# HumanCompatibleAI/imitation

Measured on NVIDIA H100. Metric: GAIL env-steps/sec (disc+gen loop), higher is better.
Workload: dtype f32

## Files before the change

imitation_b200/csrc/imb_ppo.cu:

```cuda
#include <cooperative_groups.h>
#include <stdlib.h>

#include "imb_common.cuh"
#include "imb_tile.cuh"

#ifdef IMB_PPO_TIMING
__device__ long long g_ppo_clk[24];
__device__ long long g_ppo_wclk[80];
#define PPO_TICK(i)                                  \
  do {                                               \
    if (tid == 0) {                                  \
      const long long now_ = clock64();              \
      clk_acc[i] += now_ - clk_last;                 \
      clk_last = now_;                               \
    }                                                \
  } while (0)
#define PPO_WCLK(slot)                                   \
  do {                                                   \
    if (lane == 0) wacc[slot] += clock64() - wclk0;      \
  } while (0)
#else
#define PPO_TICK(i) do {} while (0)
#define PPO_WCLK(slot) do {} while (0)
#endif
// ... 81 lines not shown
__device__ __forceinline__ float group8_sum(float v) {
  v += __shfl_xor_sync(0xffffffffu, v, 1);
  v += __shfl_xor_sync(0xffffffffu, v, 2);
  v += __shfl_xor_sync(0xffffffffu, v, 4);
  return v;
}
__device__ __forceinline__ float rcp_fast(float x) { return __fdividef(1.0f, x); }
__device__ __forceinline__ float sqrt_fast(float x) {
  float r;
  asm("sqrt.approx.f32 %0, %1;" : "=f"(r) : "f"(x));
  return r;
}

__device__ __forceinline__ float dot8r(const float (&d)[8], const float* __restrict__ b) {
  const float4 b0 = ld4(b), b1 = ld4(b + 4);
  float s0 = d[0] * b0.x, s1 = d[1] * b0.y;
  s0 = fmaf(d[2], b0.z, s0);
  s1 = fmaf(d[3], b0.w, s1);
  s0 = fmaf(d[4], b1.x, s0);
  s1 = fmaf(d[5], b1.y, s1);
  s0 = fmaf(d[6], b1.z, s0);
  s1 = fmaf(d[7], b1.w, s1);
  return s0 + s1;
}
__device__ __forceinline__ void load8(float (&d)[8], const float* __restrict__ p) {
  const float4 a = ld4(p), b = ld4(p + 4);
  d[0] = a.x, d[1] = a.y, d[2] = a.z, d[3] = a.w, d[4] = b.x, d[5] = b.y, d[6] = b.z, d[7] = b.w;
}
__device__ __forceinline__ float sum8(const float (&d)[8]) {
  return ((d[0] + d[1]) + (d[2] + d[3])) + ((d[4] + d[5]) + (d[6] + d[7]));
}

enum { RS_PG = 0, RS_V, RS_ENT, RS_CLIP, RS_KL, RS_N };
enum { AC_PG = 0, AC_V, AC_ENT, AC_CLIP, AC_KL_EPOCH, AC_LAST_PG, AC_LAST_V, AC_LAST_ENT, AC_N };

template <int NR>
__device__ __forceinline__ void ppo_stats_fold(float* __restrict__ acc, const float* __restrict__ rsl, const float inv_nb,
                                               const bool epoch_start) {
#pragma unroll 1
  for (int k = 0; k < RS_N; ++k) {
    float t = 0.f;
#pragma unroll
    for (int r = 0; r < NR; ++r) t += rsl[k * NR + r];
    t *= inv_nb;
    if (k == RS_KL) {
      acc[AC_KL_EPOCH] = epoch_start ? t : acc[AC_KL_EPOCH] + t;
    } else {
      acc[k] += t;
      if (k < RS_CLIP) acc[AC_LAST_PG + k] = t;
    }
  }
}

__device__ __forceinline__ void ppo_stats_fold_warp(float* __restrict__ acc, const float* __restrict__ rsl,
                                                    const float inv_nb, const bool epoch_start, const int lane) {
  static_assert(RS_CLIP == 3 && RS_KL == 4 && RL == 8, "fold layout");
  const float a = group8_sum(rsl[lane]), kl = group8_sum(rsl[RS_KL * RL + (lane & 7)]) * inv_nb;
  const float s_v = __shfl_sync(0xffffffffu, a, 8), s_ent = __shfl_sync(0xffffffffu, a, 16);
  const float s_clip = __shfl_sync(0xffffffffu, a, 24);
  if (lane == 0) {
    const float pg = a * inv_nb, v = s_v * inv_nb, ent = s_ent * inv_nb;
    acc[AC_PG] += pg;
    acc[AC_V] += v;
    acc[AC_ENT] += ent;
    acc[AC_CLIP] += s_clip * inv_nb;
    acc[AC_KL_EPOCH] = epoch_start ? kl : acc[AC_KL_EPOCH] + kl;
    acc[AC_LAST_PG] = pg;
    acc[AC_LAST_V] = v;
    acc[AC_LAST_ENT] = ent;
  }
}

template <int NR>
__device__ __forceinline__ float ppo_kl_part(const float* __restrict__ rsl, const float inv_nb) {
  float t = 0.f;
#pragma unroll
  for (int r = 0; r < NR; ++r) t += rsl[RS_KL * NR + r];
  return t * inv_nb;
}

__device__ __noinline__ void ppo_ev_partial(const float* __restrict__ rollout, const int64_t N, const int rw,
                                            const int col_val, const int col_ret, const int crank, double* ev,
                                            double* wred) {
  const int tid = threadIdx.x, lane = tid & 31, warp = tid >> 5;
  const double y0 = rollout[col_ret], e0 = rollout[col_ret] - rollout[col_val];
  double s[4] = {0.0, 0.0, 0.0, 0.0};
  for (int64_t i = (int64_t)crank * PT + tid; i < N; i += (int64_t)CL * PT) {
    const float y = rollout[i * rw + col_ret], e = y - rollout[i * rw + col_val];
    const double dy = (double)y - y0, de = (double)e - e0;
    s[0] += dy;
    s[1] += dy * dy;
    s[2] += de;
    s[3] += de * de;
  }
#pragma unroll
  for (int k = 0; k < 4; ++k) {
    double v = s[k];
#pragma unroll
    for (int o = 16; o > 0; o >>= 1) v += __shfl_xor_sync(0xffffffffu, v, o);
    __syncthreads();
    if (lane == 0) wred[warp] = v;
    __syncthreads();
    if (tid == 0) {
      double t = 0.0;
#pragma unroll
      for (int w = 0; w < PT / 32; ++w) t += wred[w];
      ev[k] = t;
    }
  }
}

template <typename Cluster>
__device__ __forceinline__ void ppo_stats_push(Cluster& cluster, float* box, const float* acc, const double* ev,
                                               const int crank) {
  float* dst = cluster.map_shared_rank(box, 0) + crank * 16;
#pragma unroll
  for (int k = 0; k < AC_N; ++k) dst[k] = acc[k];
#pragma unroll
  for (int k = 0; k < 4; ++k) reinterpret_cast<double*>(dst + 8)[k] = ev[k];
}

__device__ __noinline__ void ppo_stats_finish(const float* box, float* __restrict__ stats, const PpoArgs& A,
                                              const int64_t n_eval, const int64_t n_epochs, const int64_t spe,
                                              const float std, const int64_t n_updates, const bool stopped) {
  float acc[AC_N];
  double ev[4] = {0.0, 0.0, 0.0, 0.0};
#pragma unroll
  for (int k = 0; k < AC_N; ++k) acc[k] = 0.f;
  for (int c = 0; c < CL; ++c) {
    const float* a = box + c * 16;
    const double* e = reinterpret_cast<const double*>(box + c * 16 + 8);
#pragma unroll
    for (int k = 0; k < AC_N; ++k) acc[k] += a[k];
#pragma unroll
    for (int k = 0; k < 4; ++k) ev[k] += e[k];
  }
  const float ne = (float)n_eval;
  stats[IMB_PPO_STAT_ENTROPY_LOSS] = acc[AC_ENT] / ne;
  stats[IMB_PPO_STAT_PG_LOSS] = acc[AC_PG] / ne;
  stats[IMB_PPO_STAT_VALUE_LOSS] = acc[AC_V] / ne;
  stats[IMB_PPO_STAT_APPROX_KL] = acc[AC_KL_EPOCH] / (float)((n_eval - 1) % spe + 1);
  stats[IMB_PPO_STAT_CLIP_FRACTION] = acc[AC_CLIP] / ne;
  stats[IMB_PPO_STAT_LOSS] = acc[AC_LAST_PG] + A.hp.ent_coef * acc[AC_LAST_ENT] + A.hp.vf_coef * acc[AC_LAST_V];
  const double n = (double)A.n_rows;
  const double var_y = ev[1] / n - (ev[0] / n) * (ev[0] / n), var_e = ev[3] / n - (ev[2] / n) * (ev[2] / n);
  stats[IMB_PPO_STAT_EXPLAINED_VARIANCE] = var_y == 0.0 ? __int_as_float(0x7fc00000) : (float)(1.0 - var_e / var_y);
  stats[IMB_PPO_STAT_STD] = std;
  stats[IMB_PPO_STAT_N_UPDATES] = (float)n_updates;
  stats[IMB_PPO_STAT_N_STEPS] = (float)n_eval;
  stats[IMB_PPO_STAT_N_EPOCHS] = (float)n_epochs;
  stats[IMB_PPO_STAT_STOPPED] = stopped ? 1.f : 0.f;
}

struct WgradOff {
  int w1, b1, w2, b2, wa, ba, wv, bv, ls, ldo, ldh;
};
template <int NQ, int HPx>
__device__ __forceinline__ void tower_wgrad(const int tnet, const int gj, const int wq, const int h, const int Do, const int Da,
                                            const bool discrete, const WgradOff o, float* __restrict__ GP,
                                            const float* __restrict__ tH1, const float* __restrict__ tLAT,
                                            const float* __restrict__ tDZ2, const float* __restrict__ tDZ1,
                                            const float* __restrict__ XNc, const float* __restrict__ DM,
                                            const float* __restrict__ DLS, const float* __restrict__ DVAL) {
  constexpr int RLc = 8;
  constexpr int T2 = (HPx + NQ - 1) / NQ;
  float dz2[8], dz1[8], lt[8];
  if (gj < h) {
    load8(dz2, tDZ2 + gj * RLc);
    load8(dz1, tDZ1 + gj * RLc);
    load8(lt, tLAT + gj * RLc);
    {
      float r[T2];
#pragma unroll
      for (int t = 0; t < T2; ++t) {
        const int i = wq + NQ * t;
        r[t] = dot8r(dz2, tH1 + (i < HPx ? i : 0) * RLc);
      }
#pragma unroll
      for (int t = 0; t < T2; ++t) {
        const int i = wq + NQ * t;
        if (i < h) GP[o.w2 + gj * o.ldh + i] = r[t];
      }
    }
#pragma unroll
    for (int kb = 0; kb < Do; kb += 4 * NQ) {
      const int k0 = kb + wq;
      if (k0 >= Do) break;
      float r[4];
#pragma unroll
      for (int t = 0; t < 4; ++t) {
        const int k = k0 + NQ * t;
        r[t] = dot8r(dz1, XNc + (k < Do ? k : 0) * RLc);
      }
#pragma unroll
      for (int t = 0; t < 4; ++t) {
        const int k = k0 + NQ * t;
        if (k < Do) GP[o.w1 + gj * o.ldo + k] = r[t];
      }
    }
    if (tnet == 0) {
#pragma unroll
      for (int ab = 0; ab < Da; ab += 2 * NQ) {
        const int a0 = ab + wq, a1 = a0 + NQ;
        if (a0 >= Da) break;
        const float ra = dot8r(lt, DM + a0 * RLc), rb = dot8r(lt, DM + (a1 < Da ? a1 : a0) * RLc);
        GP[o.wa + a0 * o.ldh + gj] = ra;
        if (a1 < Da) GP[o.wa + a1 * o.ldh + gj] = rb;
      }
    } else if (wq == 0) {
      GP[o.wv + gj] = dot8r(lt, DVAL);
    }
    if (wq == 0) GP[o.b2 + gj] = sum8(dz2);
    if (wq == NQ - 1) GP[o.b1 + gj] = sum8(dz1);
  }
  if (wq == NQ - 1) {
    if (tnet == 0) {
#pragma unroll
      for (int tb = 0; tb < 2 * Da; tb += HPx) {
        const int t = tb + gj;
        if (t >= 2 * Da) break;
        if (t < Da) {
          load8(dz2, DM + t * RLc);
          GP[o.ba + t] = sum8(dz2);
        } else if (!discrete) {
          load8(dz2, DLS + (t - Da) * RLc);
          GP[o.ls + t - Da] = sum8(dz2);
        }
      }
    } else if (gj == 0) {
      load8(dz2, DVAL);
      GP[o.bv] = sum8(dz2);
    }
  }
}

template <int HP, int DO = 0, int DA = 0, int DISC = 0, int NORM = 0, int OPT = 0>
__global__ void __launch_bounds__(PT, 1) k_ppo_update(const PpoArgs A, float* __restrict__ g_params,
                                                      float* __restrict__ g_norm, int32_t* __restrict__ g_norm_count,
                                                      float* __restrict__ g_m, float* __restrict__ g_v,
                                                      const float* __restrict__ rollout,
                                                      const int64_t* __restrict__ perm_in,
                                                      float* __restrict__ loss_log, int64_t* __restrict__ state) {
  static_assert(HP == 32, "the warp-autonomous chain maps one lane to one hidden unit");
  namespace cg = cooperative_groups;
  cg::cluster_group cluster = cg::this_cluster();
  const int crank = (int)cluster.block_rank();
  extern __shared__ __align__(128) float smem[];
  __shared__ float red[32];
  __shared__ float bc[8];
  __shared__ __align__(8) uint64_t mbar[3];
  __shared__ __align__(8) uint64_t xbar[3];
  __shared__ float SSQ[CL];
  __shared__ float nred[PT / 32];
  __shared__ float RSL[RS_N * RL];
  __shared__ float ACC[AC_N];
  __shared__ float KLS[CL];
  __shared__ int KSTOP;
  __shared__ double EVP[4];
  __shared__ double EVW[PT / 32];
  const imb_policy_desc& pd = A.pol;
  constexpr bool SPEC = DO != 0;
  const int Do = SPEC ? DO : pd.d_obs, Da = SPEC ? DA : pd.d_act, h = SPEC ? HP : pd.hidden, NP = pd.n_params;
  const bool discrete = SPEC ? DISC != 0 : pd.discrete != 0, has_norm = SPEC ? NORM != 0 : pd.has_norm != 0;
  const PLay PL = make_play(Do, Da, h, discrete);
  const int KP = SPEC ? ppo_kp(Do) : A.KP, S = SPEC ? ppo_slice(PL) : A.S;
  constexpr int U_DO = SPEC ? DO : 8, U_H = SPEC ? HP : 8, U_DA = SPEC ? DA : 4;
  const int n_own_w = (S / 4 + 31) / 32;
  const bool tail_stats = n_own_w <= PT / 32 - 2;
  const int st0 = tail_stats ? 32 * max(n_own_w, 4) : 128, nst = PT - st0;
  const int ldo = PL.ldo, ldh = PL.ldh;
  const int da_store = discrete ? 1 : Da;
  const int col_logp = Do + da_store, col_adv = col_logp + 3, col_ret = col_logp + 4;
  const int tid = threadIdx.x, lane = tid & 31, warp = tid >> 5;
  const int rw = SPEC ? imb_row_width(Do, Da, discrete) : A.rw, RS2 = SPEC ? ppo_row_stride(rw) : A.RS2;
  auto al = [](int x) { return (x + 31) / 32 * 32; };
  const bool kl_on = OPT && A.target_kl > 0.f, vf_on = OPT && A.clip_vf > 0.f;

  int o = 0;
  float* Pm = smem + o; o += al(CL * S);
  float* Ms = smem + o; o += al(CL * S);
  float* Vs = smem + o; o += al(CL * S);
  float* GP = smem + o; o += al(CL * S);
  float* RECV = smem + o; o += al(CL * S);
  float* LOSS = smem + o; o += 32;
  const int DAP = (Da + 3) / 4 * 4;
  const int rsz = al(PR * RS2);
  float* ROWS = smem + o; o += 3 * rsz;
  const int xsz = al(KP * RL);
  float* XNo = smem + o; o += 2 * xsz;
  float* TH1 = smem + o; o += 2 * HP * RL;
  float* TLAT = smem + o; o += 2 * HP * RL;
  float* TDZ2 = smem + o; o += 2 * HP * RL;
  float* TDZ1 = smem + o; o += 2 * HP * RL;
  float* DM = smem + o; o += DAP * RL;
  float* DLS = smem + o; o += DAP * RL;
  float* MEAN = smem + o; o += DAP * RL;
  float* DVAL = smem + o; o += 32;
  float* rstat = smem + o; o += al(2 * 64 + 4);

  for (int i = tid; i < CL * S; i += PT) Pm[i] = Ms[i] = Vs[i] = GP[i] = RECV[i] = 0.f;
  for (int i = tid; i < 3 * rsz; i += PT) ROWS[i] = 0.f;
  for (int i = tid; i < 2 * xsz + 8 * HP * RL + 3 * DAP * RL + 32; i += PT) XNo[i] = 0.f;
  if (tid < 64) {
    rstat[tid] = (has_norm && tid < Do) ? g_norm[tid] : 0.f;
    rstat[64 + tid] = (has_norm && tid < Do) ? g_norm[Do + tid] : 1.f;
    LOSS[tid & 31] = 0.f;
  }
  if (tid < RS_N * RL) RSL[tid] = 0.f;
  if (tid < AC_N) ACC[tid] = 0.f;
  if (tid == 0) {
    KSTOP = 0;
    mbar_init(&mbar[0], nst);
    mbar_init(&mbar[1], nst);
    mbar_init(&mbar[2], nst);
    mbar_init(&xbar[0], 1);
    mbar_init(&xbar[1], 1);
    mbar_init(&xbar[2], 1);
    mbar_fence_init();
  }
  __syncthreads();
  for (int p = tid; p < NP; p += PT) {
    const int q = flat_to_play(pd, PL, p);
    Pm[q] = g_params[p];
    Ms[q] = g_m[p];
    Vs[q] = g_v[p];
  }
  int32_t run_count = has_norm ? *g_norm_count : 0;

  const int64_t N = A.n_rows;
  const int Ni = (int)N;
  const int mb = A.hp.batch_size;
  const int64_t steps_per_epoch = (N + mb - 1) / mb;
  const int64_t n_steps = steps_per_epoch * A.hp.n_epochs;
  int64_t adam_step = state[IMB_ST_PPO_STEP];
  const int64_t perm_draw0 = state[IMB_ST_PPO_EPOCH];
  double b1pow = pow(0.9, (double)adam_step), b2pow = pow(0.999, (double)adam_step);
  const int row0 = crank * RL;
  const WgradOff wo_p = {PL.w1[0], PL.b1[0], PL.w2[0], PL.b2[0], PL.wa, PL.ba, PL.wv, PL.bv, PL.ls, ldo, ldh};
  const WgradOff wo_v = {PL.w1[1], PL.b1[1], PL.w2[1], PL.b2[1], PL.wa, PL.ba, PL.wv, PL.bv, PL.ls, ldo, ldh};

  auto issue_gather = [&](int ep, int start, int buf) {
    if (tid < st0) return;
    const int nbx = min(mb, Ni - start);
#pragma unroll
    for (int tb = 0; tb < 2 * PR; tb += nst) {
      const int t = tb + tid - st0, r = t >> 1, half = t & 1;
      if (t >= 2 * PR) break;
      if (r >= nbx) continue;
      int64_t idx;
      if (perm_in) {
        idx = perm_in[(int64_t)ep * N + start + r];
      } else {
        const FeistelKey fk = feistel_key(A.seed, IMB_STREAM_PPO_PERM, (uint64_t)(perm_draw0 + ep), (uint64_t)N);
        idx = (int64_t)feistel_perm(fk, (uint64_t)(start + r), (uint64_t)N);
      }
      const float* src = rollout + idx * rw;
      float* dst = ROWS + buf * rsz + r * RS2;
      const int nq = rw >> 2, q0 = half ? (nq + 1) >> 1 : 0, q1 = half ? nq : (nq + 1) >> 1;
#pragma unroll
      for (int qi = 0; qi < (nq + 1) >> 1; ++qi) {
        const int q = q0 + qi;
        if (q >= q1) break;
        cp_async16(dst + 4 * q, src + 4 * q);
      }
    }
    cp_async_mbar_arrive(&mbar[buf]);
  };
  auto minibatch_stats = [&](int64_t gs2, int nbx, int gidx, int ngrp) {
    const int buf = (int)(gs2 % 3);
    float* R = ROWS + buf * rsz;
    float* XN = XNo + (int)(gs2 & 1) * xsz;
    const int gl = tid & 7;
    const float inv_nbx = 1.0f / (float)nbx;
    mbar_wait(&mbar[buf], (uint32_t)((gs2 / 3) & 1));
#pragma unroll
    for (int task0 = 0; task0 <= Do; task0 += ngrp) {
      const int task = task0 + gidx;
      const bool is_feat = task < Do, is_adv = task == Do;
      float* x = R + (is_feat ? task : col_adv);
      float v[8], s = 0.f;
#pragma unroll
      for (int i = 0; i < 8; ++i) {
        v[i] = (gl + 8 * i < nbx) ? x[(gl + 8 * i) * RS2] : 0.f;
        s += v[i];
      }
      const float bmean = group8_sum(s) * inv_nbx;
      float q = 0.f;
#pragma unroll
      for (int i = 0; i < 8; ++i) {
        const float d = (gl + 8 * i < nbx) ? v[i] - bmean : 0.f;
        q = fmaf(d, d, q);
      }
      const float ssd = group8_sum(q);
      if (is_feat) {
        float mean = 0.f, istd = 1.f;
        if (has_norm) {
          mean = rstat[task];
          float var = rstat[64 + task];
          const float bvar = ssd * inv_nbx;
          const float bn = (float)nbx, c = (float)run_count, itot = rcp_fast(c + bn), delta = bmean - mean;
          mean += delta * bn * itot;
          var *= c;
          var += bvar * bn;
          var += delta * delta * c * bn * itot;
          var *= itot;
          istd = rsqrtf(var + pd.norm_eps);
          if (gl == 0) {
            if (kl_on && crank == 0 && gs2 > 0) {
              g_norm[task] = rstat[task];
              g_norm[Do + task] = rstat[64 + task];
            }
            rstat[task] = mean;
            rstat[64 + task] = var;
          }
        }
        XN[task * RL + gl] = (row0 + gl < nbx) ? (x[(row0 + gl) * RS2] - mean) * istd : 0.f;
      } else if (is_adv) {
        float am = 0.f, ais = 1.f;
        if (A.hp.normalize_advantage && nbx > 1) {
          am = bmean;
          ais = rcp_fast(sqrt_fast(ssd / (float)(nbx - 1)) + 1e-8f);
        }
#pragma unroll
        for (int i = 0; i < 8; ++i)
          if (gl + 8 * i < nbx) x[(gl + 8 * i) * RS2] = (v[i] - am) * ais;
      }
    }
  };
  __syncthreads();
  issue_gather(0, 0, 0);
  if (n_steps > 1) issue_gather(mb >= Ni ? 1 : 0, mb >= Ni ? 0 : mb, 1);
  if (A.stats) ppo_ev_partial(rollout, N, rw, col_logp + 1, col_ret, crank, EVP, EVW);
  minibatch_stats(0, min(mb, Ni), tid >> 3, PT / 8);
  if (has_norm) run_count += min(mb, Ni);
  const uint32_t xbytes = (uint32_t)((CL - 1) * S * 4);
  const unsigned qmagic = (unsigned)(0x100000000ull / (unsigned)(S / 4)) + 1u;
  const uint32_t recv_sa = smem_u32(RECV), pm_sa = smem_u32(Pm), ssq_sa = smem_u32(SSQ);
  const uint32_t xbar0_sa = smem_u32(&xbar[0]), xbar1_sa = smem_u32(&xbar[1]), xbar2_sa = smem_u32(&xbar[2]);
  const uint32_t nbytes = (uint32_t)(CL * 4 * (kl_on ? 2 : 1));
  if (tid == 0) {
    mbar_expect_tx(&xbar[0], xbytes);
    mbar_expect_tx(&xbar[1], xbytes);
    mbar_expect_tx(&xbar[2], nbytes);
  }
  cluster.sync();

#ifdef IMB_PPO_TIMING
  long long clk_acc[16] = {0}, clk_last = clock64();
  long long wacc[10] = {0};
#endif
  int ep_now = 0, start = 0;
  for (int64_t gs = 0; gs < n_steps; ++gs) {
    const int cur = (int)(gs & 1);
    const float* Rc = ROWS + (int)(gs % 3) * rsz;
    const float* XNc = XNo + cur * xsz;
    const int nb = min(mb, Ni - start);
    const float inv_nb = 1.0f / (float)nb;
    int ep_next = ep_now, start_next = start + mb;
    if (start_next >= Ni) {
      start_next = 0;
      ++ep_next;
    }
    ++adam_step;
    if (tid == PT - 1) {
      b1pow *= 0.9;
      b2pow *= 0.999;
      bc[2 * cur] = (float)((double)A.hp.lr / (1.0 - b1pow));
      bc[2 * cur + 1] = (float)sqrt(1.0 - b2pow);
    }
    __syncthreads();
    if (kl_on && KSTOP) {
      if (tid >= st0 && gs + 1 < n_steps) mbar_wait(&mbar[(int)((gs + 1) % 3)], (uint32_t)(((gs + 1) / 3) & 1));
      if (has_norm) run_count -= min(mb, Ni - start);
      break;
    }
    PPO_TICK(0);
#ifdef IMB_PPO_TIMING
    const long long wclk0 = clock64();
#endif
    float l_pg = 0.f, l_v = 0.f, l_ent = 0.f;
    auto next_stats = [&]() {
      if (gs + 1 < n_steps) minibatch_stats(gs + 1, min(mb, Ni - start_next), (tid - st0) >> 3, nst / 8);
      PPO_WCLK(1);
    };
    if (warp >= 4) {
      if (tid >= st0) {
        if (!tail_stats) next_stats();
        if (gs + 2 < n_steps) {
          int ep2 = ep_next, start2 = start_next + mb;
          if (start2 >= Ni) {
            start2 = 0;
            ++ep2;
// ... 66 lines not shown
      st4(cLAT + j * RL + r0, make_float4(lat0, lat1, lat2, lat3));
      PPO_WCLK(4);
      float dl0 = 0.f, dl1 = 0.f, dl2 = 0.f, dl3 = 0.f;
      auto oct_sum = [&](float v) {
        v += __shfl_xor_sync(0xffffffffu, v, 4);
        v += __shfl_xor_sync(0xffffffffu, v, 2);
        v += __shfl_xor_sync(0xffffffffu, v, 1);
        return v;
      };
      if (cnet == 1) {
        const float wvj = jl ? Pm[PL.wv + j] : 0.f;
        const float p0 = lat0 * wvj, p1 = lat1 * wvj, p2 = lat2 * wvj, p3 = lat3 * wvj;
        const bool up16 = (lane & 16) != 0, up8 = (lane & 8) != 0;
        float k0 = up16 ? p2 : p0, k1 = up16 ? p3 : p1;
        k0 += __shfl_xor_sync(0xffffffffu, up16 ? p0 : p2, 16);
        k1 += __shfl_xor_sync(0xffffffffu, up16 ? p1 : p3, 16);
        float kk = up8 ? k1 : k0;
        kk += __shfl_xor_sync(0xffffffffu, up8 ? k0 : k1, 8);
        const float val = oct_sum(kk) + Pm[PL.bv];
        float dv;
        bool vin = true;
        if (vf_on) {
          const float vold = row[col_logp + 1], dvo = val - vold;
          dv = (vold + fminf(fmaxf(dvo, -A.clip_vf), A.clip_vf)) - row[col_ret];
          vin = dvo >= -A.clip_vf && dvo <= A.clip_vf;
        } else {
          dv = val - row[col_ret];
        }
        const float dval = (live && vin) ? A.hp.vf_coef * 2.0f * dv * inv_nb : 0.f;
        if (la == 0) {
          if (live) l_v = dv * dv;
          DVAL[r0 + rr] = dval;
          RSL[RS_V * RL + r0 + rr] = live ? dv * dv : 0.f;
        }
        dl0 = __shfl_sync(0xffffffffu, dval, 0) * wvj;
        dl1 = __shfl_sync(0xffffffffu, dval, 8) * wvj;
        dl2 = __shfl_sync(0xffffffffu, dval, 16) * wvj;
        dl3 = __shfl_sync(0xffffffffu, dval, 24) * wvj;
      } else {
        const float* Wa = Pm + PL.wa;
        __syncwarp();
        {
          const int asub = lane >> 2, q = lane & 3;
          const bool b0 = (lane & 1) != 0, b1 = (lane & 2) != 0;
#pragma unroll
          for (int ab = 0; ab < Da; ab += 8) {
            const int a = ab + asub, ac = a < Da ? a : 0;
            const float* wr = Wa + ac * ldh + q;
            const float* lr = cLAT + q * RL + r0;
            float s0 = 0.f, s1 = 0.f, s2 = 0.f, s3 = 0.f;
#pragma unroll
            for (int i = 0; i < HP / 4; ++i) {
              const float w = wr[4 * i];
              const float4 l4 = ld4(lr + 4 * i * RL);
              s0 = fmaf(w, l4.x, s0);
              s1 = fmaf(w, l4.y, s1);
              s2 = fmaf(w, l4.z, s2);
              s3 = fmaf(w, l4.w, s3);
            }
            float ka = b0 ? s1 : s0, kb = b0 ? s3 : s2;
            ka += __shfl_xor_sync(0xffffffffu, b0 ? s0 : s1, 1);
            kb += __shfl_xor_sync(0xffffffffu, b0 ? s2 : s3, 1);
            float kk = b1 ? kb : ka;
            kk += __shfl_xor_sync(0xffffffffu, b1 ? ka : kb, 2);
            if (a < Da) MEAN[a * RL + r0 + q] = kk + Pm[PL.ba + a];
          }
        }
        __syncwarp();
        PPO_WCLK(5);
        const float adv = pre_adv, logp_old = pre_lpo;
        float logp = 0.f, ent = 0.f;
        float r_dm = 0.f, r_dls = 0.f;
        int act = 0;
        if (gfast) {
          if (la < Da) {
            const float diff = pre_act - MEAN[la * RL + r0 + rr];
            const float d2 = diff * diff * pre_ivar;
            logp = -0.5f * d2 - pre_ls - 0.9189385332046727f;
            ent = 1.4189385332046727f + pre_ls;
            r_dm = diff * pre_ivar;
            r_dls = d2 - 1.0f;
          }
        } else if (!discrete) {
          const float* lstd = Pm + PL.ls;
          for (int a = la; a < Da; a += 8) {
            const float ls = lstd[a], ivar = __expf(-2.0f * ls);
            const float diff = row[Do + a] - MEAN[a * RL + r0 + rr];
            const float d2 = diff * diff * ivar;
            logp += -0.5f * d2 - ls - 0.9189385332046727f;
            ent += 1.4189385332046727f + ls;
            DM[a * RL + r0 + rr] = diff * ivar;
            DLS[a * RL + r0 + rr] = d2 - 1.0f;
          }
        } else {
          float mx = -INFINITY;
          for (int a = la; a < Da; a += 8) mx = fmaxf(mx, MEAN[a * RL + r0 + rr]);
          mx = fmaxf(mx, __shfl_xor_sync(0xffffffffu, mx, 4));
          mx = fmaxf(mx, __shfl_xor_sync(0xffffffffu, mx, 2));
          mx = fmaxf(mx, __shfl_xor_sync(0xffffffffu, mx, 1));
          float se = 0.f;
          for (int a = la; a < Da; a += 8) se += expf(MEAN[a * RL + r0 + rr] - mx);
          const float lse = mx + logf(oct_sum(se));
          act = (int)row[Do];
          for (int a = la; a < Da; a += 8) {
            const float lp = MEAN[a * RL + r0 + rr] - lse;
            if (a == act) logp = lp;
            ent -= expf(lp) * lp;
            DLS[a * RL + r0 + rr] = lp;
          }
        }
        logp = oct_sum(logp);
        PPO_WCLK(6);
        ent = oct_sum(ent);
        const float ratio = __expf(logp - logp_old);
        const float lo = 1.0f - A.hp.clip_range, hi = 1.0f + A.hp.clip_range;
        const float pl1 = adv * ratio, pl2 = adv * fminf(fmaxf(ratio, lo), hi);
        const bool inside = (ratio >= lo) && (ratio <= hi);
        float dl_dlogp = (inside || pl1 < pl2) ? -adv * ratio * inv_nb : 0.f;
        float dent = -A.hp.ent_coef * inv_nb;
        if (live) {
          if (la == 0) {
            l_pg = -fminf(pl1, pl2);
            l_ent = -ent;
          }
        } else {
          dl_dlogp = 0.f;
          dent = 0.f;
        }
        if (la == 0) {
          const int sr = r0 + rr;
          RSL[RS_PG * RL + sr] = live ? -fminf(pl1, pl2) : 0.f;
          RSL[RS_ENT * RL + sr] = live ? -ent : 0.f;
          RSL[RS_CLIP * RL + sr] = (live && fabsf(ratio - 1.0f) > A.hp.clip_range) ? 1.f : 0.f;
          RSL[RS_KL * RL + sr] = live ? (ratio - 1.0f) - (logp - logp_old) : 0.f;
        }
        if (gfast) {
          if (la < Da) {
            DLS[la * RL + r0 + rr] = dl_dlogp * r_dls + dent;
            DM[la * RL + r0 + rr] = dl_dlogp * r_dm;
          }
        } else if (!discrete) {
          for (int a = la; a < Da; a += 8) {
            DLS[a * RL + r0 + rr] = dl_dlogp * DLS[a * RL + r0 + rr] + dent;
            DM[a * RL + r0 + rr] = dl_dlogp * DM[a * RL + r0 + rr];
          }
        } else {
          for (int a = la; a < Da; a += 8) {
            const float lp = DLS[a * RL + r0 + rr], pp = expf(lp);
            DM[a * RL + r0 + rr] = dl_dlogp * (((a == act) ? 1.f : 0.f) - pp) + dent * (-pp * (lp + ent));
            DLS[a * RL + r0 + rr] = 0.f;
          }
        }
        __syncwarp();
        PPO_WCLK(7);
#pragma unroll U_DA
        for (int a = 0; a < Da; ++a) {
          const float waj = Wa[a * ldh + jc];
          const float4 d = ld4(DM + a * RL + r0);
          dl0 = fmaf(d.x, waj, dl0);
          dl1 = fmaf(d.y, waj, dl1);
          dl2 = fmaf(d.z, waj, dl2);
          dl3 = fmaf(d.w, waj, dl3);
        }
      }
      PPO_WCLK(2);
      st4(cDZ2 + j * RL + r0,
          make_float4(jl ? dl0 * (1.0f - lat0 * lat0) : 0.f, jl ? dl1 * (1.0f - lat1 * lat1) : 0.f,
                      jl ? dl2 * (1.0f - lat2 * lat2) : 0.f, jl ? dl3 * (1.0f - lat3 * lat3) : 0.f));
      __syncwarp();
      a0 = a1 = a2 = a3 = 0.f;
      {
        const float* wp = cW2 + jc;
#pragma unroll U_H
        for (int jj = 0; jj < h; ++jj) {
          const float w = wp[jj * ldh];
          const float4 d = ld4(cDZ2 + jj * RL + r0);
          a0 = fmaf(d.x, w, a0);
          a1 = fmaf(d.y, w, a1);
          a2 = fmaf(d.z, w, a2);
          a3 = fmaf(d.w, w, a3);
        }
      }
      st4(cDZ1 + j * RL + r0,
          make_float4(jl ? a0 * (1.f - h10 * h10) : 0.f, jl ? a1 * (1.f - h11 * h11) : 0.f,
                      jl ? a2 * (1.f - h12 * h12) : 0.f, jl ? a3 * (1.f - h13 * h13) : 0.f));
    }
    PPO_WCLK(0);
    if (warp >= 2) {
      asm volatile("bar.sync 1, 192;" ::: "memory");
      tower_wgrad<6, HP>(1, lane, warp - 2, h, Do, Da, discrete, wo_v, GP, TH1 + HP * RL, TLAT + HP * RL,
                         TDZ2 + HP * RL, TDZ1 + HP * RL, XNc, DM, DLS, DVAL);
    }
    PPO_WCLK(8);
    if (loss_log) {
      const float s_pg = block_sum(l_pg, red);
      const float s_v = block_sum(l_v, red);
      const float s_ent = block_sum(l_ent, red);
      if (tid == 0) {
        float* L0 = cluster.map_shared_rank(LOSS, 0);
        L0[crank * 3 + 0] = s_pg;
        L0[crank * 3 + 1] = s_v;
        L0[crank * 3 + 2] = s_ent;
      }
    }
    __syncthreads();
    PPO_TICK(3);
    tower_wgrad<PT / 32, HP>(0, lane, warp, h, Do, Da, discrete, wo_p, GP, TH1, TLAT, TDZ2, TDZ1, XNc, DM, DLS, DVAL);
    __syncthreads();
    PPO_TICK(7);
#pragma unroll
    for (int qb = 0; qb < (CL - 1) * (S / 4); qb += PT) {
      const int q = qb + tid;
      if (q >= (CL - 1) * (S / 4)) break;
      int qq = q + ((crank + 1) & (CL - 1)) * (S / 4);
      if (qq >= CL * S / 4) qq -= CL * S / 4;
      const int p0 = 4 * qq, owner = SPEC ? qq / (S / 4) : (int)__umulhi((unsigned)qq, qmagic);
      st_async_v4(mapa_u32(recv_sa + (uint32_t)(crank * S + (p0 - owner * S)) * 4u, owner), ld4(GP + p0),
                  mapa_u32(xbar0_sa, owner));
    }
    if (loss_log) cluster.sync();
    if (crank == 0 && tid == 0 && loss_log) {
      float pg = 0.f, vl = 0.f, el = 0.f;
      for (int c = 0; c < CL; ++c) {
        pg += LOSS[c * 3 + 0];
        vl += LOSS[c * 3 + 1];
        el += LOSS[c * 3 + 2];
      }
      pg *= inv_nb, vl *= inv_nb, el *= inv_nb;
      loss_log[gs * 4 + 0] = pg;
      loss_log[gs * 4 + 1] = vl;
      loss_log[gs * 4 + 2] = el;
      loss_log[gs * 4 + 3] = pg + A.hp.ent_coef * el + A.hp.vf_coef * vl;
    }
    PPO_TICK(8);
    if (A.stats && warp == ((tail_stats && n_own_w < 4) ? 3 : PT / 32 - 1))
      ppo_stats_fold_warp(ACC, RSL, rcp_fast((float)min(mb, Ni - start)), start == 0, threadIdx.x & 31);
    if (tail_stats && tid >= st0) {
      next_stats();
    } else {
      mbar_wait(&xbar[0], (uint32_t)(gs & 1));
      if (tid == 0) mbar_expect_tx(&xbar[0], xbytes);
      PPO_TICK(9);

      const int i0 = 4 * tid;
      const bool own = i0 < S;
      float4 g = make_float4(0.f, 0.f, 0.f, 0.f);
      float ss = 0.f;
      if (own) {
        auto part = [&](int c) { return ld4(c == crank ? GP + crank * S + i0 : RECV + c * S + i0); };
        g = part(0);
  #pragma unroll
        for (int c = 1; c < CL; ++c) {
          const float4 t = part(c);
          g.x += t.x, g.y += t.y, g.z += t.z, g.w += t.w;
        }
        ss = (g.x * g.x + g.y * g.y) + (g.z * g.z + g.w * g.w);
      }
      float my_ssq = 0.f;
      if (warp < n_own_w) {
        const float ws = warp_sum(ss);
        if (lane == 0) nred[warp] = ws;
        asm volatile("bar.sync 2, %0;" ::"r"(32 * n_own_w) : "memory");
  #pragma unroll
        for (int w = 0; w < PT / 32; ++w) my_ssq += w < n_own_w ? nred[w] : 0.f;
      }
      if (tid < CL) {
        st_async_f32(mapa_u32(ssq_sa + (uint32_t)crank * 4u, tid), my_ssq, mapa_u32(xbar2_sa, tid));
        if (kl_on)
          st_async_f32(mapa_u32(smem_u32(KLS) + (uint32_t)crank * 4u, tid), ppo_kl_part<RL>(RSL, inv_nb),
                       mapa_u32(xbar2_sa, tid));
      }
      PPO_TICK(10);
      mbar_wait(&xbar[2], (uint32_t)(gs & 1));
      if (tid == 0) mbar_expect_tx(&xbar[2], nbytes);
      PPO_TICK(11);
      bool stop = false;
      if (kl_on) {
        float kl = 0.f;
#pragma unroll
        for (int c = 0; c < CL; ++c) kl += KLS[c];
        stop = kl > 1.5f * A.target_kl;
        if (stop && tid == 0) KSTOP = (int)gs + 1;
      }

      float total = 0.f;
  #pragma unroll
      for (int c = 0; c < CL; ++c) total += SSQ[c];
      total = sqrtf(total);
      float clip = A.hp.max_grad_norm / (total + 1e-6f);
      clip = clip > 1.0f ? 1.0f : clip;
      if (own && !stop) {
        const float step_size = bc[2 * cur], inv_bc2s = rcp_fast(bc[2 * cur + 1]);
        const int q0 = crank * S + i0;
        const float4 m4 = ld4(Ms + q0), v4 = ld4(Vs + q0), p4 = ld4(Pm + q0);
        auto adam1 = [&](float gg, float& m, float& v, float& pw) {
          gg *= clip;
          m = m + (gg - m) * (1.0f - 0.9f);
          v = v * 0.999f + (1.0f - 0.999f) * gg * gg;
          pw -= step_size * __fdividef(m, fmaf(sqrt_fast(v), inv_bc2s, A.hp.adam_eps));
        };
        float4 m = m4, v = v4, pw = p4;
        adam1(g.x, m.x, v.x, pw.x);
        adam1(g.y, m.y, v.y, pw.y);
        adam1(g.z, m.z, v.z, pw.z);
        adam1(g.w, m.w, v.w, pw.w);
        st4(Ms + q0, m);
        st4(Vs + q0, v);
        st4(Pm + q0, pw);
  #pragma unroll
        for (int c = 1; c < CL; ++c) {
          const int dstc = (crank + c) & (CL - 1);
          st_async_v4(mapa_u32(pm_sa + (uint32_t)q0 * 4u, dstc), pw, mapa_u32(xbar1_sa, dstc));
        }
      }
      if (!stop) {
        mbar_wait(&xbar[1], (uint32_t)(gs & 1));
        if (tid == 0) mbar_expect_tx(&xbar[1], xbytes);
      }
      PPO_TICK(12);
    }
    if (has_norm && gs + 1 < n_steps) run_count += min(mb, Ni - start_next);
    ep_now = ep_next;
    start = start_next;
  }
  __syncthreads();
#ifdef IMB_PPO_TIMING
  if (crank == 0 && tid == 0)
    for (int i = 0; i < 16; ++i) g_ppo_clk[i] = clk_acc[i];
  if (crank == 0 && lane == 0)
    for (int i = 0; i < 10; ++i) g_ppo_wclk[i * 8 + warp] = wacc[i];
#endif

  for (int p = tid; p < NP; p += PT) {
    const int q = flat_to_play(pd, PL, p);
    if (q / S == crank) {
      g_m[p] = Ms[q];
      g_v[p] = Vs[q];
    }
  }
  const int kstop = kl_on ? KSTOP : 0;
  if (crank == 0) {
    for (int p = tid; p < NP; p += PT) g_params[p] = Pm[flat_to_play(pd, PL, p)];
    if (has_norm) {
      if (tid < Do && !(kstop && kstop < n_steps)) {
        g_norm[tid] = rstat[tid];
        g_norm[Do + tid] = rstat[64 + tid];
      }
      if (tid == 0) *g_norm_count = run_count;
    }
    if (tid == 0) {
      state[IMB_ST_PPO_STEP] = kstop ? state[IMB_ST_PPO_STEP] + (kstop - 1) : adam_step;
      state[IMB_ST_PPO_EPOCH] = perm_draw0 + (kstop ? (kstop - 1) / steps_per_epoch + 1 : A.hp.n_epochs);
    }
  }
  if (A.stats) {
    if (tid == 0) ppo_stats_push(cluster, TH1, ACC, EVP, crank);
    cluster.sync();
    if (crank == 0 && tid == 0) {
      float sd = __int_as_float(0x7fc00000);
      if (!discrete) {
// ... 296 lines not shown
```

profiles/ppo_phase_clocks.py:

```python
import ctypes
import os
import sys

import torch as th

sys.path.insert(0, os.path.dirname(os.path.dirname(os.path.abspath(__file__))))
from imitation_b200 import _desc, _lib

NAMES = ["top barrier", "-", "-", "warp chain fwd/loss/bwd", "-", "-", "-",
         "weight gradients -> GP", "push partials (7 peers)", "barrier a wait", "slice sum + norm exchange issue", "wait: slice norms landed",
         "clip + Adam (own slice) + parameter all-gather + wait", "-"]
pd = _desc.policy_desc(17, 6, False, 32, True)
N = 4096
rw = _lib.rollout_row_width(pd)
tbl = th.randn(N, rw, device="cuda")
tbl[:, 17 + 6] = -8.0 + 0.1 * th.randn(N, device="cuda")
P = (th.rand(pd.n_params, device="cuda") - 0.5) * 0.3
PN = th.cat([th.zeros(17), th.ones(17)]).cuda()
PC = th.zeros(1, dtype=th.int32, device="cuda")
M, V = th.zeros_like(P), th.zeros_like(P)
st = th.zeros(_lib.ST_WORDS, dtype=th.int64, device="cuda")
hp = _lib.PpoHparams(gamma=0.95, gae_lambda=0.95, clip_range=0.1, ent_coef=4e-6, vf_coef=0.11, max_grad_norm=0.8,
                     lr=2.6e-4, adam_eps=1e-5, n_epochs=5, batch_size=64, normalize_advantage=1)
for _ in range(3):
    _lib.ppo_update(pd, P, PN, PC, M, V, tbl, N, hp, None, 0, None, st)
th.cuda.synchronize()
_lib.lib().imb_debug_ppo_warp_clocks(None, 1)
e0, e1 = th.cuda.Event(enable_timing=True), th.cuda.Event(enable_timing=True)
e0.record()
_lib.ppo_update(pd, P, PN, PC, M, V, tbl, N, hp, None, 0, None, st)
e1.record()
th.cuda.synchronize()
steps = 5 * N // 64
print(f"launch {e0.elapsed_time(e1):.3f} ms, {e0.elapsed_time(e1) * 1e3 / steps:.2f} us/step")
out = (ctypes.c_longlong * 16)()
rc = _lib.lib().imb_debug_ppo_clocks(out)
assert rc == 0, rc
tot = sum(out[:14])
for n, c in zip(NAMES, out):
    print(f"{n:<18s} {c / steps:9.0f} cycles/step  {100.0 * c / tot:5.1f} %")
print(f"{'total':<18s} {tot / steps:9.0f} cycles/step")

w = (ctypes.c_longlong * 80)()
assert _lib.lib().imb_debug_ppo_warp_clocks(w, 0) == 0
print("per-warp cycles/step since the top barrier (CTA 0; warps 0,1 policy tower, 2,3 value tower; warps 4-7: slot 1 = "
      "next-step stats done (in the step's tail), slot 3 = prefetch issued (beside the chain)):")
for slot, name in ((1, "stats done (w4-7)"), (3, "after layer 1 | prefetch"), (4, "after layer 2"), (5, "after means (policy)"), (6, "after logp reduce"), (7, "after dM/dlogstd"),
                   (2, "after heads/loss"), (0, "chain end"), (8, "early value wgrad done (w2-7)")):
    print(f"  {name:<22s}", [round(w[slot * 8 + i] / steps) for i in range(8)])
```

Before: 2.864 million.

## Split weight-gradient work into per-layer blocks overlapped with the backward chain via named barriers

Breaks the monolithic tower weight-gradient routine into layer-2, head and layer-1 pieces. Warps 4-7 compute value dW2, policy head and policy dW2 gradients as soon as named-barrier arrivals from the chain warps signal that the inputs are ready. Warps 2-3 compute value dW1. After the block-wide barrier only policy dW1/b1 remains. This is meant to shorten the serialized weight-gradient phase by overlapping it with the chain. In exchange it adds named-barrier arrive/sync pairs and an uneven load across warps.

```diff
diff --git a/imitation_b200/csrc/imb_ppo.cu b/imitation_b200/csrc/imb_ppo.cu
--- a/imitation_b200/csrc/imb_ppo.cu
+++ b/imitation_b200/csrc/imb_ppo.cu
@@ -257,86 +257,110 @@
   stats[IMB_PPO_STAT_STOPPED] = stopped ? 1.f : 0.f;
 }
 
-struct WgradOff {
-  int w1, b1, w2, b2, wa, ba, wv, bv, ls, ldo, ldh;
-};
+
 template <int NQ, int HPx>
-__device__ __forceinline__ void tower_wgrad(const int tnet, const int gj, const int wq, const int h, const int Do, const int Da,
-                                            const bool discrete, const WgradOff o, float* __restrict__ GP,
-                                            const float* __restrict__ tH1, const float* __restrict__ tLAT,
-                                            const float* __restrict__ tDZ2, const float* __restrict__ tDZ1,
-                                            const float* __restrict__ XNc, const float* __restrict__ DM,
-                                            const float* __restrict__ DLS, const float* __restrict__ DVAL) {
+__device__ __forceinline__ void wgrad_layer2(const bool value, const int gj, const int wq, const int h, const int w2,
+                                             const int b2, const int ldh, const int wv, const int bv,
+                                             float* __restrict__ GP, const float* __restrict__ tH1,
+                                             const float* __restrict__ tLAT, const float* __restrict__ tDZ2,
+                                             const float* __restrict__ DVAL) {
   constexpr int RLc = 8;
   constexpr int T2 = (HPx + NQ - 1) / NQ;
-  float dz2[8], dz1[8], lt[8];
+  float dz2[8];
   if (gj < h) {
     load8(dz2, tDZ2 + gj * RLc);
-    load8(dz1, tDZ1 + gj * RLc);
-    load8(lt, tLAT + gj * RLc);
-    {
-      float r[T2];
-#pragma unroll
-      for (int t = 0; t < T2; ++t) {
-        const int i = wq + NQ * t;
-        r[t] = dot8r(dz2, tH1 + (i < HPx ? i : 0) * RLc);
-      }
-#pragma unroll
-      for (int t = 0; t < T2; ++t) {
-        const int i = wq + NQ * t;
-        if (i < h) GP[o.w2 + gj * o.ldh + i] = r[t];
-      }
-    }
-#pragma unroll
-    for (int kb = 0; kb < Do; kb += 4 * NQ) {
-      const int k0 = kb + wq;
-      if (k0 >= Do) break;
-      float r[4];
-#pragma unroll
-      for (int t = 0; t < 4; ++t) {
-        const int k = k0 + NQ * t;
-        r[t] = dot8r(dz1, XNc + (k < Do ? k : 0) * RLc);
-      }
-#pragma unroll
-      for (int t = 0; t < 4; ++t) {
-        const int k = k0 + NQ * t;
-        if (k < Do) GP[o.w1 + gj * o.ldo + k] = r[t];
-      }
-    }
-    if (tnet == 0) {
-#pragma unroll
-      for (int ab = 0; ab < Da; ab += 2 * NQ) {
-        const int a0 = ab + wq, a1 = a0 + NQ;
-        if (a0 >= Da) break;
-        const float ra = dot8r(lt, DM + a0 * RLc), rb = dot8r(lt, DM + (a1 < Da ? a1 : a0) * RLc);
-        GP[o.wa + a0 * o.ldh + gj] = ra;
-        if (a1 < Da) GP[o.wa + a1 * o.ldh + gj] = rb;
-      }
-    } else if (wq == 0) {
-      GP[o.wv + gj] = dot8r(lt, DVAL);
-    }
-    if (wq == 0) GP[o.b2 + gj] = sum8(dz2);
-    if (wq == NQ - 1) GP[o.b1 + gj] = sum8(dz1);
+    float r[T2];
+#pragma unroll
+    for (int t = 0; t < T2; ++t) {
+      const int i = wq + NQ * t;
+      r[t] = dot8r(dz2, tH1 + (i < HPx ? i : 0) * RLc);
+    }
+    float rv = 0.f;
+    if (value && wq == NQ - 1) {
+      float lt[8];
+      load8(lt, tLAT + gj * RLc);
+      rv = dot8r(lt, DVAL);
+    }
+#pragma unroll
+    for (int t = 0; t < T2; ++t) {
+      const int i = wq + NQ * t;
+      if (i < h) GP[w2 + gj * ldh + i] = r[t];
+    }
+    if (wq == 0) GP[b2 + gj] = sum8(dz2);
+    if (value && wq == NQ - 1) GP[wv + gj] = rv;
+  }
+  if (value && wq == NQ - 1 && gj == 0) {
+    load8(dz2, DVAL);
+    GP[bv] = sum8(dz2);
+  }
+}
+
+template <int NQ>
+__device__ __forceinline__ void wgrad_layer1(const int gj, const int wq, const int h, const int Do, const int w1,
+                                             const int b1, const int ldo, float* __restrict__ GP,
+                                             const float* __restrict__ tDZ1, const float* __restrict__ XNc) {
+  constexpr int RLc = 8;
+  if (gj >= h) return;
+  float dz1[8];
+  load8(dz1, tDZ1 + gj * RLc);
+#pragma unroll
+  for (int kb = 0; kb < Do; kb += 4 * NQ) {
+    const int k0 = kb + wq;
+    if (k0 >= Do) break;
+    float r[4];
+#pragma unroll
+    for (int t = 0; t < 4; ++t) {
+      const int k = k0 + NQ * t;
+      r[t] = dot8r(dz1, XNc + (k < Do ? k : 0) * RLc);
+    }
+#pragma unroll
+    for (int t = 0; t < 4; ++t) {
+      const int k = k0 + NQ * t;
+      if (k < Do) GP[w1 + gj * ldo + k] = r[t];
+    }
+  }
+  if (wq == NQ - 1) GP[b1 + gj] = sum8(dz1);
+}
+
+template <int NQ, int HPx>
+__device__ __forceinline__ void wgrad_head(const int gj, const int wq, const int h, const int Da, const bool discrete,
+                                           const PLay& L, float* __restrict__ GP, const float* __restrict__ tLAT,
+                                           const float* __restrict__ DM, const float* __restrict__ DLS) {
+  constexpr int RLc = 8;
+  float d[8];
+  if (gj < h) {
+    load8(d, tLAT + gj * RLc);
+#pragma unroll
+    for (int ab = 0; ab < Da; ab += 2 * NQ) {
+      const int a0 = ab + wq, a1 = a0 + NQ;
+      if (a0 >= Da) break;
+      const float ra = dot8r(d, DM + a0 * RLc), rb = dot8r(d, DM + (a1 < Da ? a1 : a0) * RLc);
+      GP[L.wa + a0 * L.ldh + gj] = ra;
+      if (a1 < Da) GP[L.wa + a1 * L.ldh + gj] = rb;
+    }
   }
   if (wq == NQ - 1) {
-    if (tnet == 0) {
-#pragma unroll
-      for (int tb = 0; tb < 2 * Da; tb += HPx) {
-        const int t = tb + gj;
-        if (t >= 2 * Da) break;
-        if (t < Da) {
-          load8(dz2, DM + t * RLc);
-          GP[o.ba + t] = sum8(dz2);
-        } else if (!discrete) {
-          load8(dz2, DLS + (t - Da) * RLc);
-          GP[o.ls + t - Da] = sum8(dz2);
-        }
-      }
-    } else if (gj == 0) {
-      load8(dz2, DVAL);
-      GP[o.bv] = sum8(dz2);
-    }
-  }
+#pragma unroll
+    for (int tb = 0; tb < 2 * Da; tb += HPx) {
+      const int t = tb + gj;
+      if (t >= 2 * Da) break;
+      if (t < Da) {
+        load8(d, DM + t * RLc);
+        GP[L.ba + t] = sum8(d);
+      } else if (!discrete) {
+        load8(d, DLS + (t - Da) * RLc);
+        GP[L.ls + t - Da] = sum8(d);
+      }
+    }
+  }
+}
+
+enum { BAR_VDZ2 = 3, BAR_PHEAD = 4, BAR_PDZ2 = 5, BAR_VDZ1 = 6 };
+__device__ __forceinline__ void bar_arrive(const int id, const int n) {
+  asm volatile("bar.arrive %0, %1;" ::"r"(id), "r"(n) : "memory");
+}
+__device__ __forceinline__ void bar_sync(const int id, const int n) {
+  asm volatile("bar.sync %0, %1;" ::"r"(id), "r"(n) : "memory");
 }
 
 template <int HP, int DO = 0, int DA = 0, int DISC = 0, int NORM = 0, int OPT = 0>
@@ -441,8 +465,6 @@
   const int64_t perm_draw0 = state[IMB_ST_PPO_EPOCH];
   double b1pow = pow(0.9, (double)adam_step), b2pow = pow(0.999, (double)adam_step);
   const int row0 = crank * RL;
-  const WgradOff wo_p = {PL.w1[0], PL.b1[0], PL.w2[0], PL.b2[0], PL.wa, PL.ba, PL.wv, PL.bv, PL.ls, ldo, ldh};
-  const WgradOff wo_v = {PL.w1[1], PL.b1[1], PL.w2[1], PL.b2[1], PL.wa, PL.ba, PL.wv, PL.bv, PL.ls, ldo, ldh};
 
   auto issue_gather = [&](int ep, int start, int buf) {
     if (tid < st0) return;
@@ -815,6 +837,7 @@
           }
         }
         __syncwarp();
+        bar_arrive(BAR_PHEAD, 192);
         PPO_WCLK(7);
 #pragma unroll U_DA
         for (int a = 0; a < Da; ++a) {
@@ -831,6 +854,7 @@
           make_float4(jl ? dl0 * (1.0f - lat0 * lat0) : 0.f, jl ? dl1 * (1.0f - lat1 * lat1) : 0.f,
                       jl ? dl2 * (1.0f - lat2 * lat2) : 0.f, jl ? dl3 * (1.0f - lat3 * lat3) : 0.f));
       __syncwarp();
+      bar_arrive(cnet ? BAR_VDZ2 : BAR_PDZ2, 192);
       a0 = a1 = a2 = a3 = 0.f;
       {
         const float* wp = cW2 + jc;
@@ -849,10 +873,20 @@
                       jl ? a2 * (1.f - h12 * h12) : 0.f, jl ? a3 * (1.f - h13 * h13) : 0.f));
     }
     PPO_WCLK(0);
-    if (warp >= 2) {
-      asm volatile("bar.sync 1, 192;" ::: "memory");
-      tower_wgrad<6, HP>(1, lane, warp - 2, h, Do, Da, discrete, wo_v, GP, TH1 + HP * RL, TLAT + HP * RL,
-                         TDZ2 + HP * RL, TDZ1 + HP * RL, XNc, DM, DLS, DVAL);
+    if (warp >= 4) {
+      bar_sync(BAR_VDZ2, 192);
+      wgrad_layer2<4, HP>(true, lane, warp - 4, h, PL.w2[1], PL.b2[1], ldh, PL.wv, PL.bv, GP, TH1 + HP * RL,
+                          TLAT + HP * RL, TDZ2 + HP * RL, DVAL);
+      PPO_WCLK(9);
+      bar_sync(BAR_PHEAD, 192);
+      wgrad_head<4, HP>(lane, warp - 4, h, Da, discrete, PL, GP, TLAT, DM, DLS);
+      PPO_WCLK(7);
+      bar_sync(BAR_PDZ2, 192);
+      wgrad_layer2<4, HP>(false, lane, warp - 4, h, PL.w2[0], PL.b2[0], ldh, 0, 0, GP, TH1, TLAT, TDZ2, DVAL);
+    } else if (warp >= 2) {
+      bar_sync(BAR_VDZ1, 64);
+      wgrad_layer1<2>(lane, warp - 2, h, Do, PL.w1[1], PL.b1[1], ldo, GP, TDZ1 + HP * RL, XNc);
+      PPO_WCLK(9);
     }
     PPO_WCLK(8);
     if (loss_log) {
@@ -868,7 +902,8 @@
     }
     __syncthreads();
     PPO_TICK(3);
-    tower_wgrad<PT / 32, HP>(0, lane, warp, h, Do, Da, discrete, wo_p, GP, TH1, TLAT, TDZ2, TDZ1, XNc, DM, DLS, DVAL);
+    if (warp >= 2) PPO_WCLK(6);
+    wgrad_layer1<PT / 32>(lane, warp, h, Do, PL.w1[0], PL.b1[0], ldo, GP, TDZ1, XNc);
     __syncthreads();
     PPO_TICK(7);
 #pragma unroll
diff --git a/profiles/ppo_phase_clocks.py b/profiles/ppo_phase_clocks.py
--- a/profiles/ppo_phase_clocks.py
+++ b/profiles/ppo_phase_clocks.py
@@ -7,8 +7,8 @@
 sys.path.insert(0, os.path.dirname(os.path.dirname(os.path.abspath(__file__))))
 from imitation_b200 import _desc, _lib
 
-NAMES = ["top barrier", "-", "-", "warp chain fwd/loss/bwd", "-", "-", "-",
-         "weight gradients -> GP", "push partials (7 peers)", "barrier a wait", "slice sum + norm exchange issue", "wait: slice norms landed",
+NAMES = ["top barrier", "-", "-", "chain + early wgrad blocks", "-", "-", "-",
+         "policy dW1/b1 -> GP", "push partials (7 peers)", "barrier a wait", "slice sum + norm exchange issue", "wait: slice norms landed",
          "clip + Adam (own slice) + parameter all-gather + wait", "-"]
 pd = _desc.policy_desc(17, 6, False, 32, True)
 N = 4096
@@ -44,7 +44,13 @@
 w = (ctypes.c_longlong * 80)()
 assert _lib.lib().imb_debug_ppo_warp_clocks(w, 0) == 0
 print("per-warp cycles/step since the top barrier (CTA 0; warps 0,1 policy tower, 2,3 value tower; warps 4-7: slot 1 = "
-      "next-step stats done (in the step's tail), slot 3 = prefetch issued (beside the chain)):")
-for slot, name in ((1, "stats done (w4-7)"), (3, "after layer 1 | prefetch"), (4, "after layer 2"), (5, "after means (policy)"), (6, "after logp reduce"), (7, "after dM/dlogstd"),
-                   (2, "after heads/loss"), (0, "chain end"), (8, "early value wgrad done (w2-7)")):
-    print(f"  {name:<22s}", [round(w[slot * 8 + i] / steps) for i in range(8)])
+      "next-step stats done (in the step's tail), slot 3 = prefetch issued (beside the chain); early weight-gradient "
+      "blocks: value dW2, policy head and policy dW2 on warps 4-7, value dW1 on warps 2,3).\n"
+      "Each warp counts from its own read of the clock after the top barrier; the rows of warps that reach that barrier "
+      "early (4-7) run ahead of the others' by about their wait there: align them on the post-chain barrier row, which "
+      "thread 0 passes at the 'chain + early wgrad blocks' total above.")
+for slot, name in ((1, "stats done (w4-7)"), (3, "after layer 1 | prefetch"), (4, "after layer 2"), (5, "after means (policy)"), (6, "after logp reduce"),
+                   (7, "after dM/dlogstd | head wgrad (w4-7)"), (2, "after heads/loss"), (0, "chain end"),
+                   (9, "value dW1 (w2,3) | value dW2 (w4-7)"), (8, "early wgrad blocks done (w2-7)"),
+                   (6, "after logp reduce | post-chain barrier (w2-7)")):
+    print(f"  {name:<36s}", [round(w[slot * 8 + i] / steps) for i in range(8)])
```

New measurement: 3.081 million (median of 6 runs). +7.6%, better.
